# nekStab/neklab

Measured on AMD Instinct MI355X. Metric: linop matvecs/sec + Arnoldi iter time, E=10k N=7, 1/2/4/8 GPU, higher is better.
Workload: dtype f64

## Files before the change

neklab_amd/csrc/lns.hip:

```cpp
#include <cmath>
#include <functional>
#include <map>
#include <string>

#include "internal.h"

using namespace nlg;

namespace {

constexpr int NT = 256;
constexpr int NB = 512;

struct F3 {
    double *p[3];
};
struct CF3 {
    const double *p[3];
};
__device__ __forceinline__ int64_t lane_lo(int64_t ld) { return (int64_t)blockIdx.y * ld; }
__device__ __forceinline__ F3 lane_f3(F3 a, int64_t lo) {
#pragma unroll
    for (int c = 0; c < 3; ++c)
        if (a.p[c]) a.p[c] += lo;
// ... 1974 lines not shown
    hipStream_t st = m->ctx->stream;
    const int dim = m->dim, nl = L.nl;
    const int64_t ld = L.ld();
    const double dt = op->dt, b0 = op->adv_b0;
    double **unew = op->ubuf[2];
    NLG_LAUNCH(k_axpy1, lgrid(grid_for(m->lpn), nl), dim3(NT), 0, st, m->lpn, op->p, (const double *)op->pr_x, 1.0, ld);
    const bool fg = sem_opgradt_has_fg(m);
    NLG_TRY(sem_opgradt(m, op->pr_x, op->gp, fg, nullptr, nullptr, nl, ld, ld));
    NLG_TRY(sem_gs(m, op->gp, dim, nullptr, fg ? LAYOUT_FG : LAYOUT_NAT, nl, ld, 0));
    const bool fused = op->d_filt && op->filt_fused;
    if (!fused) {
        CF3 wt = {{m->d_mbinv[0], m->d_mbinv[1], m->d_mbinv[2]}};
        const bool wb = fg && op->maskb_v && m->d_maskb_fg && m->d_binv_fg;
        if (wb) wt.p[0] = m->d_binv_fg;
        if (fg)
            launch_nf(dim, k_axpy_w<1, true>, k_axpy_w<2, true>, k_axpy_w<3, true>, lgrid(grid_for(m->lvn), nl), st, m->lvn, f3(unew, dim), cf3(op->gp, dim),
                      wt, dt / b0, ld, (const int *)m->d_slot_fg, m->np1, wb ? (const unsigned char *)m->d_maskb_fg : (const unsigned char *)nullptr);
        else
            launch_nf(dim, k_axpy_w<1>, k_axpy_w<2>, k_axpy_w<3>, lgrid(grid_for(m->lvn), nl), st, m->lvn, f3(unew, dim), cf3(op->gp, dim), wt, dt / b0,
                      ld, (const int *)nullptr, 1, (const unsigned char *)nullptr);
    }
    if (op->d_filt) {
        double *fl[4] = {unew[0], unew[1], dim == 3 ? unew[2] : op->tbuf[0], op->tbuf[0]};
        const int nf = dim + (op->cfg.ifheat ? 1 : 0);
        if (fused)
            NLG_TRY(sem_filter(m, op->d_filt, fl, nf, nl, ld, op->gp, m->d_mbinv, dt / b0, fg ? (const int *)m->d_slot_fg : nullptr));
        else
            NLG_TRY(sem_filter(m, op->d_filt, fl, nf, nl, ld));
    }
    NLG_HIP(hipGetLastError());
    rotate3(op->ubuf);
    op->st_steps += nl;
    return 0;
}

int advance(const Lanes &L) {
    NLG_TRY(adv_a(L));
    NLG_TRY(helm_solve(L, L.op->adv_k, L.op->adv_h2));
    NLG_TRY(adv_b(L));
    NLG_TRY(pres_solve(L, L.op->dt / L.op->adv_b0));
    return adv_c(L);
}

int reset_state(nlg_linop *op, int nl) {
    nlg_mesh *m = op->mesh;
    NLG_TRY(slab_ensure(op, nl));
    lane_bind(op);
    const int64_t nlev = (int64_t)(6 * m->dim + (op->cfg.ifheat ? 6 : 0)) * m->lvs;
    for (int v = 0; v < nl; ++v) NLG_HIP(hipMemsetAsync(op->slab + (size_t)v * (size_t)op->slab_ld, 0, sizeof(double) * (size_t)nlev, m->ctx->stream));
    return 0;
}

int begin_run(nlg_linop *op, int nl) {
    NLG_TRY(reset_state(op, nl));
    op->istep = 0;
    op->nproj = 0;
    for (int v = 0; v < kMaxLanes; ++v) op->lane_viters[v] = op->lane_piters[v] = 0;
    op->orbit_end_valid = op->upo_fdot_valid = false;
    return 0;
}

int load_state(nlg_linop *op, int lane, const nlg_vec *v, int irst) {
    nlg_mesh *m = op->mesh;
    hipStream_t st = m->ctx->stream;
    for (int c = 0; c < m->dim; ++c)
        NLG_HIP(hipMemcpyAsync(at_lane(op, op->ubuf[0][c], lane), v->vel(c, irst), sizeof(double) * (size_t)m->lvn, hipMemcpyDeviceToDevice, st));
    NLG_HIP(hipMemcpyAsync(at_lane(op, op->p, lane), v->pr(irst), sizeof(double) * (size_t)m->lpn, hipMemcpyDeviceToDevice, st));
    if (op->cfg.ifheat)
        NLG_HIP(hipMemcpyAsync(at_lane(op, op->tbuf[0], lane), v->theta(0, irst), sizeof(double) * (size_t)m->lvn, hipMemcpyDeviceToDevice, st));
    return 0;
}

int store_state(nlg_linop *op, int lane, nlg_vec *v, int irst) {
    nlg_mesh *m = op->mesh;
    hipStream_t st = m->ctx->stream;
    for (int c = 0; c < m->dim; ++c)
        NLG_HIP(hipMemcpyAsync(v->vel(c, irst), at_lane(op, op->ubuf[0][c], lane), sizeof(double) * (size_t)m->lvn, hipMemcpyDeviceToDevice, st));
    NLG_HIP(hipMemcpyAsync(v->pr(irst), at_lane(op, op->p, lane), sizeof(double) * (size_t)m->lpn, hipMemcpyDeviceToDevice, st));
    if (op->cfg.ifheat)
        NLG_HIP(hipMemcpyAsync(v->theta(0, irst), at_lane(op, op->tbuf[0], lane), sizeof(double) * (size_t)m->lvn, hipMemcpyDeviceToDevice, st));
    return 0;
}

int state_minus_x0(nlg_linop *op, int lane, double c, nlg_vec *out) {
    nlg_mesh *m = op->mesh;
    const int dim = m->dim;
    DdtArgs A;
    memset(&A, 0, sizeof(A));
    for (int f = 0; f <= dim; ++f) {
        const bool pr = f == dim;
        A.out[f] = pr ? out->pr() : out->vel(f), A.n[f] = pr ? m->lpn : m->lvn;
        A.src[f][0] = at_lane(op, pr ? op->p : op->ubuf[0][f], lane), A.c[f][0] = c;
        A.src[f][1] = pr ? op->baseflow->pr() : op->baseflow->vel(f), A.c[f][1] = -c;
    }
    NLG_LAUNCH(k_bdf_ddt, dim3(grid_for(m->lvn), dim + 1), dim3(NT), 0, m->ctx->stream, A);
    NLG_HIP(hipGetLastError());
    return 0;
}

enum { FDOT_START = 0, FDOT_PRE, FDOT_END };
int capture_fdot(nlg_linop *op, int lane, int phase) {
    nlg_mesh *m = op->mesh;
    const int dim = m->dim;
    const double idt = 1.0 / op->dt;
    if (phase == FDOT_START) return state_minus_x0(op, lane, idt, op->upo_f0);
    nlg_vec *o = op->upo_fT;
    DdtArgs A;
    memset(&A, 0, sizeof(A));
    for (int c = 0; c < dim; ++c) A.out[c] = o->vel(c), A.n[c] = m->lvn;
    A.out[dim] = o->pr(), A.n[dim] = m->lpn;
    if (phase == FDOT_PRE) {
        const int k = std::min(op->nsteps, op->cfg.torder);
        for (int c = 0; c < dim; ++c)
            for (int j = 0; j < k; ++j) A.src[c][j] = at_lane(op, op->ubuf[j][c], lane), A.c[c][j] = -BDF_C[k][j] * idt;
    } else {
        const int k = std::min(op->nsteps, op->cfg.torder);
        A.acc = 1;
        for (int c = 0; c < dim; ++c) A.src[c][0] = at_lane(op, op->ubuf[0][c], lane), A.c[c][0] = BDF_B0[k] * idt;
        A.src[dim][0] = at_lane(op, op->pr_x, lane), A.c[dim][0] = idt;
        op->upo_fdot_valid = true;
    }
    NLG_LAUNCH(k_bdf_ddt, dim3(grid_for(m->lvn), dim + 1), dim3(NT), 0, m->ctx->stream, A);
    NLG_HIP(hipGetLastError());
    return 0;
}

template <typename Hook>
int run_steps(const Lanes &L, int fdot_lane, Hook after_step) {
    nlg_linop *op = L.op;
    for (int istep = 1; istep <= op->nsteps; ++istep) {
        if (fdot_lane >= 0 && istep == op->nsteps) NLG_TRY(capture_fdot(op, fdot_lane, FDOT_PRE));
        NLG_TRY(advance(L));
        if (fdot_lane >= 0 && istep == 1) NLG_TRY(capture_fdot(op, fdot_lane, FDOT_START));
        NLG_TRY(after_step(istep));
    }
    if (fdot_lane >= 0) NLG_TRY(capture_fdot(op, fdot_lane, FDOT_END));
    return 0;
}
int run_steps(const Lanes &L, int fdot_lane = -1) {
    return run_steps(L, fdot_lane, [](int) { return 0; });
}

int project_lines(nlg_linop *op, const ProjLines &P, int nf, F3 f, int s, unsigned mask) {
    nlg_mesh *m = op->mesh;
    hipStream_t st = m->ctx->stream;
    const int64_t nl = P.nlines, ld = op->slab_ld, tld = P.tld;
    const dim3 g((unsigned)((nl + NT / 64 - 1) / (NT / 64)), (unsigned)s);
    const int *off = P.off, *idx = P.idx, *gs = P.gslot;
    const double *cv = P.cv, *sv = P.sv, *iden = P.iden, *glob = P.glob;
    if (!gs) {
        launch_nf(nf, k_proj_alpha<1>, k_proj_alpha<2>, k_proj_alpha<3>, g, st, nl, off, idx, P.weight, cv, sv, tld, iden, f, ld, mask);
    } else {
        const int64_t cnt = P.nglob * s * 2 * nf;
        NLG_HIP(hipMemsetAsync(P.glob, 0, sizeof(double) * (size_t)cnt, st));
        if (nl > 0)
            launch_nf(nf, k_proj_sums<1>, k_proj_sums<2>, k_proj_sums<3>, g, st, nl, off, idx, gs, P.weight, cv, sv, tld,
                      CF3{{f.p[0], f.p[1], f.p[2]}}, ld, mask, P.glob);
        NLG_TRY(allreduce_sum(m->ctx, P.glob, (int)cnt));
        if (nl > 0) launch_nf(nf, k_proj_apply<1>, k_proj_apply<2>, k_proj_apply<3>, g, st, nl, off, idx, gs, cv, sv, tld, iden, glob, f, ld, mask);
    }
    NLG_HIP(hipGetLastError());
    return 0;
}

int project_alpha(nlg_linop *op, int s, int slot, unsigned mask) {
    if (op->proj_v.nlines == 0) return 0;
    NLG_TRY(project_lines(op, op->proj_v, op->mesh->dim, f3(op->ubuf[slot], op->mesh->dim), s, mask));
    const ProjLines &Pp = op->proj_p;
    if ((Pp.gslot || Pp.nlines > 0) && slot == 0) NLG_TRY(project_lines(op, Pp, 1, F3{{op->p, nullptr, nullptr}}, s, mask));
    return 0;
}

int do_matvec_block(nlg_linop *op, int s, const nlg_vec *const *vin, nlg_vec *const *vout, int adjoint) {
    NLG_CHECK(op && vin && vout, "exptA block matvec: NULL argument");
    NLG_CHECK(s >= 1 && s <= kMaxLanes, "exptA block matvec: %d vectors unsupported (1..%d)", s, kMaxLanes);
    NLG_CHECK(op->inited, "exptA block matvec: nlg_linop_init has not been called");
    NLG_NO_OTD(op, "exptA matvec");
    if (op->orbit) {
        NLG_CHECK(s <= kMaxLanes - 1, "exptA block matvec: orbit mode advances the base flow as one of the %d lanes, %d vectors unsupported (1..%d)",
                  kMaxLanes, s, kMaxLanes - 1);
        NLG_CHECK(!adjoint, "exptA rmatvec: orbit mode has no adjoint (the adjoint of a time-dependent linearisation needs U(T - t); nlg_linop_set_orbit)");
    }
    nlg_mesh *m = op->mesh;
    const int want_scal = op->cfg.ifheat ? 1 : 0;
    for (int v = 0; v < s; ++v) {
        NLG_CHECK(vin[v] && vout[v] && vin[v]->mesh == m && vout[v]->mesh == m, "exptA block matvec: vector %d NULL or on a different mesh", v);
        NLG_CHECK(vin[v]->nscal == want_scal && vout[v]->nscal == want_scal, "exptA block matvec: vector %d carries %d scalars, the operator %d", v,
                  vin[v]->nscal, want_scal);
        NLG_CHECK(op->cfg.no_history || (vin[v]->lorder >= op->cfg.torder && vout[v]->lorder >= op->cfg.torder), "exptA block matvec: vector lorder < time order");
        for (int u = 0; u < s; ++u) NLG_CHECK(vin[v] != vout[u], "exptA block matvec: an input vector is also an output vector");
        for (int u = 0; u < v; ++u) NLG_CHECK(vout[v] != vout[u], "exptA block matvec: the same output vector twice");
    }
    const int nrst = op->cfg.no_history ? 0 : op->cfg.torder - 1;
    const int nl = op->orbit ? s + 1 : s, lb = op->orbit ? s : -1;
    NLG_CHECK(op->proj_lanes == 0 || s <= op->proj_lanes, "exptA block matvec: %d vectors on an operator with %d wavenumber lanes (nlg_linop_set_projection_lanes)", s,
              op->proj_lanes);
    const unsigned all = (1u << s) - 1u;
    NLG_TRY(begin_run(op, nl));
    for (int v = 0; v < s; ++v) NLG_TRY(load_state(op, v, vin[v], 0));
    NLG_TRY(project_alpha(op, s, 0, all));
    if (lb >= 0) NLG_TRY(load_state(op, lb, op->baseflow, 0));
    Lanes L{op, nl, lb};
    L.adjoint = adjoint;
    NLG_TRY(run_steps(L, lb, [&](int istep) -> int {
        if (istep <= nrst) {
            unsigned replayed = 0;
            for (int v = 0; v < s; ++v)
                if (vin[v]->nrst > 0) {
                    NLG_TRY(load_state(op, v, vin[v], istep));
                    replayed |= 1u << v;
                }
            if (replayed) NLG_TRY(project_alpha(op, s, 0, replayed));
        }
        return 0;
    }));
    for (int slot = 0; slot < 3; ++slot) NLG_TRY(project_alpha(op, s, slot, all));
    for (int v = 0; v < s; ++v) {
        NLG_TRY(nlg_vec_zero(vout[v]));
        NLG_TRY(store_state(op, v, vout[v], 0));
    }
    if (lb >= 0) {
        NLG_TRY(nlg_vec_zero(op->orbit_end));
        NLG_TRY(store_state(op, lb, op->orbit_end, 0));
        op->orbit_end_valid = true;
    }
    for (int irst = 1; irst <= nrst; ++irst) {
        NLG_TRY(advance(L));
        for (int v = 0; v < s; ++v) {
            NLG_TRY(store_state(op, v, vout[v], irst));
            vout[v]->nrst = std::max(vout[v]->nrst, irst);
        }
    }
    op->st_matvecs += s;
    return 0;
}

int do_matvec(nlg_linop *op, const nlg_vec *vin, nlg_vec *vout, int adjoint) {
    NLG_CHECK(op && vin && vout, "exptA matvec: NULL argument");
    NLG_CHECK(op->inited, "exptA matvec: nlg_linop_init has not been called (reference: exptA%%init(), 1cyl.usr:20)");
    nlg_mesh *m = op->mesh;
    NLG_CHECK(vin->mesh == m && vout->mesh == m,
              "exptA matvec: vector on a different mesh (reference: type_error, exponential_propagator.f90:53-58)");
    NLG_CHECK(vin->nscal == (op->cfg.ifheat ? 1 : 0) && vout->nscal == vin->nscal,
              "exptA matvec: the vectors carry %d scalar(s), the operator expects %d (cfg.ifheat)", vin->nscal, op->cfg.ifheat ? 1 : 0);
    NLG_CHECK(op->cfg.no_history || (vin->lorder >= op->cfg.torder && vout->lorder >= op->cfg.torder),
              "exptA matvec: vector lorder %d < time order %d", vin->lorder, op->cfg.torder);
    NLG_CHECK(vin != vout, "exptA matvec: vec_in and vec_out must be distinct (intent(in) / intent(out))");
    return do_matvec_block(op, 1, &vin, &vout, adjoint);
}

int do_integrate_forced_block(nlg_linop *op, int s, const nlg_vec *const *ic, const nlg_vec *const *f_re, const nlg_vec *const *f_im, double omega,
                              int adjoint, nlg_vec *const *vout) {
    NLG_CHECK(op && f_re && vout, "integrate_forced: NULL argument");
    NLG_CHECK(s >= 1 && s <= kMaxLanes, "integrate_forced: %d forcings unsupported (1..%d)", s, kMaxLanes);
    NLG_CHECK(op->inited, "integrate_forced: nlg_linop_init has not been called");
    NLG_NO_OTD(op, "integrate_forced");
    NLG_CHECK(!op->orbit, "integrate_forced: not available in orbit mode (the forced response about a time-periodic base flow is not built; nlg_linop_set_orbit)");
    NLG_CHECK(op->proj_lanes == 0, "integrate_forced: not available on an operator with wavenumber lanes (a forced run does not project; nlg_linop_set_projection_lanes)");
    nlg_mesh *m = op->mesh;
    Lanes L{op, s};
    for (int v = 0; v < s; ++v) {
        NLG_CHECK(f_re[v] && vout[v], "integrate_forced: NULL argument (forcing or output of lane %d)", v);
        L.f_re[v] = f_re[v];
        L.f_im[v] = f_im ? f_im[v] : nullptr;
    }
    for (int v = 0; v < s; ++v) {
        const nlg_vec *icv = ic ? ic[v] : nullptr;
        NLG_CHECK(L.f_re[v]->mesh == m && vout[v]->mesh == m && (!icv || icv->mesh == m) && (!L.f_im[v] || L.f_im[v]->mesh == m),
                  "integrate_forced: vector on a different mesh");
        for (int u = 0; u < s; ++u)
            NLG_CHECK(vout[v] != L.f_re[u] && vout[v] != L.f_im[u] && !(ic && vout[v] == ic[u]), "integrate_forced: the output must be distinct from the inputs");
        for (int u = 0; u < v; ++u) NLG_CHECK(vout[v] != vout[u], "integrate_forced: the same output vector twice");
        NLG_CHECK(L.f_re[v]->nscal == 0 && vout[v]->nscal == 0, "integrate_forced: scalar (temperature) coupling is not built yet");
    }
    hipStream_t st = m->ctx->stream;
    NLG_TRY(begin_run(op, s));
    for (int v = 0; v < s; ++v) {
        NLG_HIP(hipMemsetAsync(at_lane(op, op->p, v), 0, sizeof(double) * (size_t)m->lps, st));
        if (ic && ic[v]) NLG_TRY(load_state(op, v, ic[v], 0));
    }
    L.adjoint = adjoint;
    L.omega = omega, L.sign = adjoint ? -1.0 : 1.0;
    NLG_TRY(run_steps(L));
    for (int v = 0; v < s; ++v) {
        NLG_TRY(nlg_vec_zero(vout[v]));
        NLG_TRY(store_state(op, v, vout[v], 0));
    }
    return 0;
}

int do_integrate_forced(nlg_linop *op, const nlg_vec *ic, const nlg_vec *f_re, const nlg_vec *f_im, double omega, int adjoint, nlg_vec *vout) {
    NLG_CHECK(op && f_re && vout, "integrate_forced: NULL argument");
    return do_integrate_forced_block(op, 1, &ic, &f_re, &f_im, omega, adjoint, &vout);
}

int do_nonlinear_map(nlg_linop *op, const nlg_vec *vin, nlg_vec *vout) {
    NLG_CHECK(op && vin && vout, "nonlinear_map: NULL argument");
    NLG_NO_OTD(op, "nonlinear_map");
    nlg_mesh *m = op->mesh;
    NLG_CHECK(vin->mesh == m && vout->mesh == m, "nonlinear_map: vector on a different mesh (reference: type_error, fixed_point.f90:31-36)");
    NLG_CHECK(vin->nscal == (op->cfg.ifheat ? 1 : 0) && vout->nscal == vin->nscal,
              "nonlinear_map: the vectors carry %d scalar(s), the operator expects %d (cfg.ifheat)", vin->nscal, op->cfg.ifheat ? 1 : 0);
    NLG_CHECK(vin != vout, "nonlinear_map: vec_in and vec_out must be distinct");
    NLG_CHECK(!op->orbit, "nonlinear_map: the operator is in orbit mode and holds X0 as its base flow (use a second operator, or nlg_linop_set_orbit(op, NULL, 0))");
    NLG_TRY(nlg_vec_copy(op->baseflow, vin));
// ... 787 lines not shown
```

neklab_amd/csrc/vec.hip:

```cpp
#include <algorithm>

#include "internal.h"

using namespace nlg;

namespace {

constexpr int NT = 256;

__device__ __forceinline__ double wave_sum(double v) {
#pragma unroll
    for (int o = 32; o > 0; o >>= 1) v += __shfl_down(v, o, 64);
    return v;
}

__device__ __forceinline__ double block_sum(double v, double *sm) {
    v = wave_sum(v);
    const int lane = threadIdx.x & 63, wid = threadIdx.x >> 6;
    __syncthreads();
    if (lane == 0) sm[wid] = v;
    __syncthreads();
    double r = 0.0;
    if (threadIdx.x == 0) {
        const int nw = (blockDim.x + 63) >> 6;
// ... 83 lines not shown
    const int64_t beg = blockIdx.x * per, end = (beg + per < n2) ? beg + per : n2;
    const int64_t off = (int64_t)c * lvs;
    double2 *w2 = reinterpret_cast<double2 *>(w + off);
    const double2 *v2 = reinterpret_cast<const double2 *>(v + off);
    const double2 *t2 = reinterpret_cast<const double2 *>(fT + off);
    const double2 *f2 = reinterpret_cast<const double2 *>(f0 + off);
    const double2 *m2 = reinterpret_cast<const double2 *>(bm1);
    double acc = 0.0;
    for (int64_t i = beg + threadIdx.x; i < end; i += NT) {
        const double2 vv = v2[i], tv = t2[i];
        double2 wv = w2[i];
        wv.x = __dadd_rn(__dadd_rn(wv.x, -vv.x), __dmul_rn(t, tv.x));
        wv.y = __dadd_rn(__dadd_rn(wv.y, -vv.y), __dmul_rn(t, tv.y));
        w2[i] = wv;
        if (ip) {
            const double2 fv = f2[i], mv = m2[i];
            acc += vv.x * fv.x * mv.x + vv.y * fv.y * mv.y;
        }
    }
    if (ip) {
        const double s = block_sum(acc, sm);
        if (threadIdx.x == 0) partial[c * nblk + blockIdx.x] = s;
    }
}

__global__ __launch_bounds__(NT) void k_reduce_rows(const double *partial, int nper, double *out, int accumulate,
                                                    double *out2) {
    __shared__ double sm[4];
    const double *p = partial + (int64_t)blockIdx.x * nper;
    double acc = 0.0;
    for (int i = threadIdx.x; i < nper; i += NT) acc += p[i];
    const double s = block_sum(acc, sm);
    if (threadIdx.x == 0) {
        out[blockIdx.x] = s;
        if (accumulate) out2[blockIdx.x] += s;
    }
}

template <int KB>
__global__ __launch_bounds__(NT) void k_block_dot(const double *V, int64_t vstride, int k, const double *w,
                                                  const double *bm1, int64_t lvs, int nblk, int nper,
                                                  double *partial) {
    __shared__ double sm[4 * KB];
    const int c = blockIdx.y;
    const int j0 = blockIdx.z * KB;
    const int kc = (k - j0 < KB) ? (k - j0) : KB;
    const int64_t n2 = lvs >> 1;
    const int64_t per = (n2 + nblk - 1) / nblk;
    const int64_t beg = blockIdx.x * per, end = (beg + per < n2) ? beg + per : n2;
    const double2 *w2 = reinterpret_cast<const double2 *>(w + c * lvs);
    const double2 *m2 = reinterpret_cast<const double2 *>(bm1);
    const double2 *v2[KB];
#pragma unroll
    for (int j = 0; j < KB; ++j) {
        const int jj = (j < kc) ? j : 0;
        v2[j] = reinterpret_cast<const double2 *>(V + (int64_t)(j0 + jj) * vstride + c * lvs);
    }
    double acc[KB];
#pragma unroll
    for (int j = 0; j < KB; ++j) acc[j] = 0.0;
    for (int64_t i = beg + threadIdx.x; i < end; i += NT) {
        const double2 wv = w2[i], mv = m2[i];
        const double x0 = wv.x * mv.x, x1 = wv.y * mv.y;
        double2 vv[KB];
#pragma unroll
        for (int j = 0; j < KB; ++j) vv[j] = v2[j][i];
#pragma unroll
        for (int j = 0; j < KB; ++j) acc[j] += vv[j].x * x0 + vv[j].y * x1;
    }
    const int lane = threadIdx.x & 63, wid = threadIdx.x >> 6;
#pragma unroll
    for (int j = 0; j < KB; ++j) {
        const double s = wave_sum(acc[j]);
        if (lane == 0) sm[wid * KB + j] = s;
    }
    __syncthreads();
    if (threadIdx.x < kc) {
        const int j = threadIdx.x;
        const double s = sm[j] + sm[KB + j] + sm[2 * KB + j] + sm[3 * KB + j];
        partial[(int64_t)(j0 + j) * nper + c * nblk + blockIdx.x] = s;
    }
}

template <int KMAX>
__global__ __launch_bounds__(NT) void k_block_axpy_dot(const double *__restrict__ V, int64_t vstride, int k,
                                                       const double *__restrict__ h, double *__restrict__ w,
                                                       const double *__restrict__ bm1, int64_t lvs, int64_t nv,
                                                       double *__restrict__ partial) {
    __shared__ double sh[KMAX];
    __shared__ double sm[4][KMAX];
    for (int j = threadIdx.x; j < KMAX; j += NT) sh[j] = j < k ? h[j] : 0.0;
    __syncthreads();
    double acc[KMAX];
#pragma unroll
    for (int j = 0; j < KMAX; ++j) acc[j] = 0.0;
    for (int64_t i = blockIdx.x * (int64_t)NT + threadIdx.x; i < nv; i += (int64_t)gridDim.x * NT) {
        double v[KMAX];
#pragma unroll
        for (int j = 0; j < KMAX; ++j) v[j] = j < k ? V[(int64_t)j * vstride + i] : 0.0;
        double s = 0.0;
#pragma unroll
        for (int j = 0; j < KMAX; ++j) s += sh[j] * v[j];
        const double wn = w[i] - s;
        w[i] = wn;
        const double x = wn * bm1[i % lvs];
#pragma unroll
        for (int j = 0; j < KMAX; ++j) acc[j] += v[j] * x;
    }
    const int lane = threadIdx.x & 63, wid = threadIdx.x >> 6;
#pragma unroll
    for (int j = 0; j < KMAX; ++j) {
        const double t = wave_sum(acc[j]);
        if (lane == 0) sm[wid][j] = t;
    }
    __syncthreads();
    if (threadIdx.x < k) {
        const int j = threadIdx.x;
        partial[(int64_t)j * gridDim.x + blockIdx.x] = (sm[0][j] + sm[1][j]) + (sm[2][j] + sm[3][j]);
    }
}

template <int KH>
__global__ __launch_bounds__(NT) void k_block_axpy_dot2(const double *__restrict__ V, int64_t vstride, int k,
                                                        const double *__restrict__ h, double *__restrict__ w,
                                                        const double *__restrict__ bm1, int64_t lvs, int64_t nv,
                                                        double *__restrict__ partial) {
    extern __shared__ double dyn2[];
    double *sh = dyn2;
    double *stash = dyn2 + 2 * KH;
    __shared__ double sm[4][2 * KH];
    for (int j = threadIdx.x; j < 2 * KH; j += NT) sh[j] = j < k ? h[j] : 0.0;
    __syncthreads();
    double acc0[KH], acc1[KH];
#pragma unroll
    for (int j = 0; j < KH; ++j) acc0[j] = 0.0, acc1[j] = 0.0;
    double *mine = stash + threadIdx.x;
    for (int64_t i = blockIdx.x * (int64_t)NT + threadIdx.x; i < nv; i += (int64_t)gridDim.x * NT) {
        double v[KH];
#pragma unroll
        for (int j = 0; j < KH; ++j) v[j] = KH + j < k ? V[(int64_t)(KH + j) * vstride + i] : 0.0;
        double s1 = 0.0;
#pragma unroll
        for (int j = 0; j < KH; ++j) {
            s1 += sh[KH + j] * v[j];
            mine[j * NT] = v[j];
        }
#pragma unroll
        for (int j = 0; j < KH; ++j) v[j] = V[(int64_t)j * vstride + i];
        double s0 = 0.0;
#pragma unroll
        for (int j = 0; j < KH; ++j) s0 += sh[j] * v[j];
        const double wn = w[i] - (s0 + s1);
        w[i] = wn;
        const double x = wn * bm1[i % lvs];
#pragma unroll
        for (int j = 0; j < KH; ++j) {
            acc0[j] += v[j] * x;
            acc1[j] += mine[j * NT] * x;
        }
    }
    const int lane = threadIdx.x & 63, wid = threadIdx.x >> 6;
#pragma unroll
    for (int j = 0; j < KH; ++j) {
        const double t0 = wave_sum(acc0[j]), t1 = wave_sum(acc1[j]);
        if (lane == 0) sm[wid][j] = t0, sm[wid][KH + j] = t1;
    }
    __syncthreads();
    if (threadIdx.x < k) {
        const int j = threadIdx.x;
        partial[(int64_t)j * gridDim.x + blockIdx.x] = (sm[0][j] + sm[1][j]) + (sm[2][j] + sm[3][j]);
    }
}

__global__ __launch_bounds__(NT) void k_block_axpy(const double *V, int64_t vstride, int k, const double *h, double *w,
                                                   int64_t n2, int nrst, int64_t blk2, int consistent, double sign,
                                                   const double *hh) {
    extern __shared__ double sh0[];
    double *sh1 = sh0 + k;
    for (int j = threadIdx.x; j < k; j += NT) {
        sh0[j] = h[j];
        sh1[j] = hh ? hh[j] : h[j];
    }
    __syncthreads();
    double2 *w2 = reinterpret_cast<double2 *>(w);
    for (int64_t i = blockIdx.x * (int64_t)NT + threadIdx.x; i < n2; i += (int64_t)gridDim.x * NT) {
        const double *sh = (hh && i >= blk2) ? sh1 : sh0;
        double s0 = 0.0, s1 = 0.0;
        const double2 *v = reinterpret_cast<const double2 *>(V) + i;
        const int64_t vs2 = vstride >> 1;
        int j = 0;
        for (; j + 8 <= k; j += 8) {
            double2 t[8];
#pragma unroll
            for (int u = 0; u < 8; ++u) t[u] = v[(int64_t)(j + u) * vs2];
#pragma unroll
            for (int u = 0; u < 8; ++u) {
                s0 += sh[j + u] * t[u].x;
                s1 += sh[j + u] * t[u].y;
            }
        }
        for (; j < k; ++j) {
            const double2 t = v[(int64_t)j * vs2];
            s0 += sh[j] * t.x;
            s1 += sh[j] * t.y;
        }
        double2 wv = w2[i];
        wv.x += sign * s0;
        wv.y += sign * s1;
        w2[i] = wv;
        for (int r = 1; r <= nrst; ++r) {
            double c0 = s0, c1 = s1;
            if (consistent) {
                c0 = c1 = 0.0;
                for (int jj = 0; jj < k; ++jj) {
                    const double2 t = v[(int64_t)jj * vs2 + r * blk2];
                    c0 += sh[jj] * t.x;
                    c1 += sh[jj] * t.y;
                }
            }
            double2 rv = w2[i + r * blk2];
            rv.x += sign * c0;
            rv.y += sign * c1;
            w2[i + r * blk2] = rv;
        }
    }
}

template <int KB, int S>
__global__ __launch_bounds__(NT) void k_block_dot_s(const double *V, int64_t vstride, int k, const double *W, int64_t wstride,
                                                    const double *bm1, int64_t lvs, int nblk, int nper, double *partial) {
    __shared__ double sm[4 * KB * S];
    const int c = blockIdx.y;
    const int j0 = blockIdx.z * KB;
    const int kc = (k - j0 < KB) ? (k - j0) : KB;
    const int64_t n2 = lvs >> 1;
    const int64_t per = (n2 + nblk - 1) / nblk;
    const int64_t beg = blockIdx.x * per, end = (beg + per < n2) ? beg + per : n2;
    const double2 *m2 = reinterpret_cast<const double2 *>(bm1);
    const double2 *v2[KB];
#pragma unroll
    for (int j = 0; j < KB; ++j) {
        const int jj = (j < kc) ? j : 0;
        v2[j] = reinterpret_cast<const double2 *>(V + (int64_t)(j0 + jj) * vstride + c * lvs);
    }
    double acc[KB][S];
#pragma unroll
    for (int j = 0; j < KB; ++j)
#pragma unroll
        for (int v = 0; v < S; ++v) acc[j][v] = 0.0;
    for (int64_t i = beg + threadIdx.x; i < end; i += NT) {
        const double2 mv = m2[i];
        double x0[S], x1[S];
#pragma unroll
        for (int v = 0; v < S; ++v) {
            const double2 wv = reinterpret_cast<const double2 *>(W + (int64_t)v * wstride + c * lvs)[i];
            x0[v] = wv.x * mv.x;
            x1[v] = wv.y * mv.y;
        }
        double2 vv[KB];
#pragma unroll
        for (int j = 0; j < KB; ++j) vv[j] = v2[j][i];
#pragma unroll
        for (int j = 0; j < KB; ++j)
#pragma unroll
            for (int v = 0; v < S; ++v) acc[j][v] += vv[j].x * x0[v] + vv[j].y * x1[v];
    }
    const int lane = threadIdx.x & 63, wid = threadIdx.x >> 6;
#pragma unroll
    for (int j = 0; j < KB; ++j)
#pragma unroll
        for (int v = 0; v < S; ++v) {
            const double t = wave_sum(acc[j][v]);
            if (lane == 0) sm[wid * KB * S + j * S + v] = t;
        }
    __syncthreads();
    if (threadIdx.x < kc * S) {
        const int q = threadIdx.x;
        const double t = (sm[q] + sm[KB * S + q]) + (sm[2 * KB * S + q] + sm[3 * KB * S + q]);
        partial[((int64_t)j0 * S + q) * nper + c * nblk + blockIdx.x] = t;
    }
}

template <int S>
__global__ __launch_bounds__(NT) void k_block_axpy_s(const double *V, int64_t vstride, int k, const double *h, const double *hh,
                                                     double *W, int64_t wstride, int64_t n2, int64_t blk2, double sign) {
    extern __shared__ double shs[];
    double *sh0 = shs, *sh1 = shs + (size_t)k * S;
    for (int j = threadIdx.x; j < k * S; j += NT) {
        sh0[j] = h[j];
        sh1[j] = hh ? hh[j] : h[j];
    }
    __syncthreads();
    const int64_t vs2 = vstride >> 1, ws2 = wstride >> 1;
    double2 *w2 = reinterpret_cast<double2 *>(W);
    for (int64_t i = blockIdx.x * (int64_t)NT + threadIdx.x; i < n2; i += (int64_t)gridDim.x * NT) {
        const double *sh = (hh && i >= blk2) ? sh1 : sh0;
        const double2 *v = reinterpret_cast<const double2 *>(V) + i;
        double s0[S], s1[S];
#pragma unroll
        for (int q = 0; q < S; ++q) s0[q] = s1[q] = 0.0;
        int j = 0;
        for (; j + 8 <= k; j += 8) {
            double2 t[8];
#pragma unroll
            for (int u = 0; u < 8; ++u) t[u] = v[(int64_t)(j + u) * vs2];
#pragma unroll
            for (int u = 0; u < 8; ++u)
// ... 557 lines not shown
    hipError_t e = hipMalloc(&b->d, bytes);
    if (e != hipSuccess) {
        delete b;
        set_error("nlg_basis_create: hipMalloc(%zu bytes) failed: %s", bytes, hipGetErrorString(e));
        return 1;
    }
    NLG_HIP(hipMemsetAsync(b->d, 0, bytes, mesh->ctx->stream));
    NLG_HIP(hipMalloc(&b->d_h, sizeof(double) * (size_t)(3 * nvec + 16)));
    NLG_HIP(hipMemsetAsync(b->d_h, 0, sizeof(double) * (size_t)(3 * nvec + 16), mesh->ctx->stream));
    NLG_TRY(reduce_ws_reserve(mesh->ctx, nvec + 8));
    b->views.resize(nvec);
    for (int i = 0; i < nvec; ++i) {
        nlg_vec *v = new nlg_vec();
        v->mesh = mesh;
        v->nscal = nscal;
        v->lorder = lorder;
        v->ncomp = ncomp;
        v->main_len = main_len;
        v->total_len = b->stride;
        v->d = b->d + (int64_t)i * b->stride;
        v->owns = false;
        b->views[i] = v;
    }
    *out = b;
    return 0;
}

int nlg_basis_destroy(nlg_basis *b) {
    if (!b) return 0;
    for (auto *v : b->views) delete v;
    if (b->d) hipFree(b->d);
    if (b->d_h) hipFree(b->d_h);
    if (b->d_hb) hipFree(b->d_hb);
    delete b;
    return 0;
}

int nlg_basis_vec(nlg_basis *b, int i, nlg_vec **out) {
    NLG_CHECK(b && out, "nlg_basis_vec: NULL argument");
    NLG_CHECK(i >= 0 && i < b->nvec, "nlg_basis_vec: index %d out of range [0,%d)", i, b->nvec);
    *out = b->views[i];
    return 0;
}

}

namespace nlg {

static int reduce_rows_all(nlg_ctx *ctx, int rows, int per, double *out, double *acc) {
    hipStream_t st = ctx->stream;
    if (ctx->distributed()) {
        NLG_LAUNCH(k_reduce_rows, dim3(rows), dim3(NT), 0, st, ctx->d_partial, per, out, 0, (double *)nullptr);
        NLG_TRY(allreduce_sum(ctx, out, rows));
        if (acc) NLG_LAUNCH(k_vadd, dim3((rows + 255) / 256), dim3(256), 0, st, acc, out, rows);
    } else {
        ++g_collectives;
        NLG_LAUNCH(k_reduce_rows, dim3(rows), dim3(NT), 0, st, ctx->d_partial, per, out, acc ? 1 : 0, acc);
    }
    return 0;
}

int basis_block_dot_dev(const nlg_basis *b, int k, const nlg_vec *w, double *d_out, double *d_acc) {
    nlg_ctx *ctx = b->mesh->ctx;
    const nlg_vec *v0 = b->views[0];
    constexpr int KB = 8;
    const int nblk = dot_nblk(v0);
    const int nper = nblk * v0->ncomp;
    NLG_TRY(reduce_ws_reserve(ctx, k));
    ProfScope ps(ctx, P_BLOCKDOT);
    NLG_LAUNCH(k_block_dot<KB>, dim3(nblk, v0->ncomp, (k + KB - 1) / KB), dim3(NT), 0, ctx->stream, b->d,
                       b->stride, k, w->d, b->mesh->d_bm1, b->mesh->lvs, nblk, nper, ctx->d_partial);
    NLG_TRY(reduce_rows_all(ctx, k, nper, d_out, d_acc));
    NLG_HIP(hipGetLastError());
    return 0;
}

int basis_block_axpy_dev(const nlg_basis *b, int k, const double *d_h, nlg_vec *w, double sign, const double *d_hh,
                         bool main_only) {
    nlg_ctx *ctx = b->mesh->ctx;
    const int64_t n2 = w->main_len / 2;
    ProfScope ps(ctx, P_BLOCKAXPY);
    if (g_axpby_consistent) {
        const int64_t n2all = main_only ? n2 : n2 * (1 + w->nrst);
        NLG_LAUNCH(k_block_axpy, dim3(grid_for(n2all)), dim3(NT), sizeof(double) * 2 * k, ctx->stream, b->d, b->stride,
                           k, d_h, w->d, n2all, 0, n2, 0, sign, d_hh);
    } else {
        NLG_LAUNCH(k_block_axpy, dim3(grid_for(n2)), dim3(NT), sizeof(double) * 2 * k, ctx->stream, b->d, b->stride, k,
                           d_h, w->d, n2, w->nrst, n2, 0, sign, (const double *)nullptr);
    }
    NLG_HIP(hipGetLastError());
    return 0;
}

int basis_cgs2_dev(nlg_basis *b, int k, nlg_vec *w) {
    nlg_ctx *ctx = b->mesh->ctx;
    double *h = b->d_h, *h2 = b->d_h + b->nvec + 8;
    if (k > 0) {
        NLG_TRY(basis_block_dot_dev(b, k, w, h, nullptr));
        if (g_axpby_consistent) {
            if (k >= 24) {
                const nlg_vec *v0 = b->views[0];
                const int kf = std::min(k, 128);
                const int k0 = k - kf;
                const int64_t nv = (int64_t)v0->ncomp * b->mesh->lvs;
                const int G = 256;
                NLG_TRY(reduce_ws_reserve(ctx, k));
                if (k0 > 0) NLG_TRY(basis_block_axpy_dev(b, k0, h, w, -1.0, nullptr, true));
                const double *Vf = b->d + (int64_t)k0 * b->stride;
                {
                    ProfScope ps(ctx, P_AXPYDOT);
                    if (kf > 64) {
                        constexpr size_t lds2 = sizeof(double) * (2 * 64 + 64 * NT);
                        static bool attr_set = false;
                        if (!attr_set) {
                            NLG_HIP(hipFuncSetAttribute(reinterpret_cast<const void *>(&k_block_axpy_dot2<64>), hipFuncAttributeMaxDynamicSharedMemorySize, (int)lds2));
                            attr_set = true;
                        }
                        NLG_LAUNCH(k_block_axpy_dot2<64>, dim3(G), dim3(NT), lds2, ctx->stream, Vf, b->stride, kf,
                                           (const double *)(h + k0), w->d, (const double *)b->mesh->d_bm1, b->mesh->lvs, nv, ctx->d_partial);
                    } else {
                        NLG_LAUNCH(k_block_axpy_dot<64>, dim3(G), dim3(NT), 0, ctx->stream, Vf, b->stride, kf,
                                           (const double *)(h + k0), w->d, (const double *)b->mesh->d_bm1, b->mesh->lvs, nv, ctx->d_partial);
                    }
                }
                {
                    ProfScope ps(ctx, P_BLOCKAXPY);
                    const int64_t np2 = (w->main_len - nv) / 2;
                    if (np2 > 0)
                        NLG_LAUNCH(k_block_axpy, dim3(grid_for(np2)), dim3(NT), sizeof(double) * 2 * kf, ctx->stream,
                                           Vf + nv, b->stride, kf, (const double *)(h + k0), w->d + nv, np2, 0, np2, 0, -1.0,
                                           (const double *)nullptr);
                }
                NLG_TRY(reduce_rows_all(ctx, kf, G, h2 + k0, h + k0));
                if (k0 > 0) NLG_TRY(basis_block_dot_dev(b, k0, w, h2, h));
            } else {
                NLG_TRY(basis_block_axpy_dev(b, k, h, w, -1.0, nullptr, true));
                NLG_TRY(basis_block_dot_dev(b, k, w, h2, h));
            }
            NLG_TRY(basis_block_axpy_dev(b, k, h2, w, -1.0, h, false));
        } else {
            NLG_TRY(basis_block_axpy_dev(b, k, h, w, -1.0));
            NLG_TRY(basis_block_dot_dev(b, k, w, h2, h));
            NLG_TRY(basis_block_axpy_dev(b, k, h2, w, -1.0));
        }
    }
    const int nblk = dot_nblk(w);
    NLG_LAUNCH(k_dot_partial, dim3(nblk, w->ncomp), dim3(NT), 0, ctx->stream, w->d, w->d, b->mesh->d_bm1,
                       b->mesh->lvs, nblk, ctx->d_partial);
    NLG_TRY(reduce_rows_all(ctx, 1, nblk * w->ncomp, h + k, nullptr));
    const int64_t n2 = w->main_len * (1 + w->nrst) / 2;
    NLG_LAUNCH(k_scal_dev, dim3(grid_for(n2)), dim3(NT), 0, ctx->stream, reinterpret_cast<double2 *>(w->d),
                       h + k, 0, n2);
    NLG_HIP(hipGetLastError());
    return 0;
}

int basis_cgs2_batch_dev(int s, nlg_basis *const *b, int k, nlg_vec *const *w) {
    nlg_basis *b0 = b[0];
    nlg_mesh *m = b0->mesh;
    nlg_ctx *ctx = m->ctx;
    hipStream_t st = ctx->stream;
    if (!b0->d_hb) NLG_HIP(hipMalloc(&b0->d_hb, sizeof(double) * ((size_t)2 * b0->nvec * 4 + 64)));
    double *H1 = b0->d_hb, *Q = H1 + (size_t)s * k, *H2 = b0->d_hb + (size_t)b0->nvec * 4 + 8;
    if (!g_axpby_consistent) {
        for (int l = 0; l < s; ++l) {
            NLG_TRY(basis_cgs2_dev(b[l], k, w[l]));
            if (k > 0) NLG_HIP(hipMemcpyAsync(H1 + (size_t)l * k, b[l]->d_h, sizeof(double) * k, hipMemcpyDeviceToDevice, st));
            NLG_HIP(hipMemcpyAsync(Q + l, b[l]->d_h + k, sizeof(double), hipMemcpyDeviceToDevice, st));
        }
        return 0;
    }
    LaneVW P;
    int nrst = 0;
    for (int l = 0; l < kMaxLanes; ++l) {
        const int u = l < s ? l : 0;
        P.V[l] = b[u]->d, P.w[l] = w[u]->d, P.nrst[l] = w[u]->nrst;
        nrst = std::max(nrst, w[u]->nrst);
    }
    const nlg_vec *v0 = b0->views[0];
    constexpr int KB = 8;
    const int nblk = dot_nblk(v0), nper = nblk * v0->ncomp;
    const int64_t n2 = v0->main_len / 2;
    NLG_TRY(reduce_ws_reserve(ctx, s * std::max(k, 1)));
    auto dot = [&](double *out, double *acc) -> int {
        ProfScope ps(ctx, P_BLOCKDOT);
        NLG_LAUNCH(k_lane_block_dot<KB>, dim3(nblk, v0->ncomp * s, (k + KB - 1) / KB), dim3(NT), 0, st, P, b0->stride, k, v0->ncomp,
                   (const double *)m->d_bm1, m->lvs, nblk, nper, ctx->d_partial);
        return reduce_rows_all(ctx, s * k, nper, out, acc);
    };
    auto axpy = [&](const double *h, const double *hh, bool main_only) -> int {
        ProfScope ps(ctx, P_BLOCKAXPY);
        const int64_t n2all = main_only ? n2 : n2 * (1 + nrst);
        NLG_LAUNCH(k_lane_block_axpy, dim3(grid_for(n2all), s), dim3(NT), sizeof(double) * 2 * k, st, P, b0->stride, k, h, hh, n2, (int)main_only, -1.0);
        return 0;
    };
    if (k > 0) {
        NLG_TRY(dot(H1, nullptr));
        NLG_TRY(axpy(H1, nullptr, true));
        NLG_TRY(dot(H2, H1));
        NLG_TRY(axpy(H2, H1, false));
    }
    NLG_LAUNCH(k_lane_dot_partial, dim3(nblk, v0->ncomp, s), dim3(NT), 0, st, P, (const double *)m->d_bm1, m->lvs, nblk, nper, ctx->d_partial);
    NLG_TRY(reduce_rows_all(ctx, s, nper, Q, nullptr));
    NLG_LAUNCH(k_lane_scal_dev, dim3(grid_for(n2 * (1 + nrst)), s), dim3(NT), 0, st, P, (const double *)Q, n2);
    NLG_HIP(hipGetLastError());
    return 0;
}

}

extern "C" {

int nlg_basis_cgs2_batch(int s, nlg_basis *const *b, int k, nlg_vec *const *w, double *h, int ldh, double *beta) {
    NLG_CHECK(b && w && h && beta, "nlg_basis_cgs2_batch: NULL argument");
    NLG_CHECK(s >= 1 && s <= kMaxLanes, "nlg_basis_cgs2_batch: %d lanes unsupported (1..%d)", s, kMaxLanes);
    for (int l = 0; l < s; ++l) NLG_CHECK(b[l] && w[l], "nlg_basis_cgs2_batch: NULL basis or vector in lane %d", l);
    NLG_CHECK(k >= 0 && k <= b[0]->nvec, "nlg_basis_cgs2_batch: k=%d out of range [0,%d]", k, b[0]->nvec);
// ... 217 lines not shown
```

Measured before the change: 24.34.

## Fuse CGS2 norm and scaling into block-axpy epilogues; trim output zeroing

Adds a dedicated four-sweep CGS2 path for k between 24 and 128. It computes the first projection with a dot-only variant of the axpy-dot kernel, then fuses the second axpy with the weighted norm reduction, and folds the normalization scaling into the axpy over the remaining (restart) region. This removes separate dot/scale passes over the vector. Separately, zeroing of output vectors before store_state now memsets only the regions not overwritten by the subsequent copies, rather than the whole vector. The risk is subtle reordering of reductions changing rounding, and more code paths to keep consistent.

```diff
diff --git a/neklab_amd/csrc/lns.hip b/neklab_amd/csrc/lns.hip
--- a/neklab_amd/csrc/lns.hip
+++ b/neklab_amd/csrc/lns.hip
@@ -2080,6 +2080,18 @@
     return 0;
 }
 
+int reset_for_store(nlg_linop *op, nlg_vec *v, int nrst) {
+    nlg_mesh *m = op->mesh;
+    hipStream_t st = m->ctx->stream;
+    v->nrst = 0;
+    const int64_t beg = (int64_t)(1 + nrst) * v->main_len;
+    if (beg < v->total_len) NLG_HIP(hipMemsetAsync(v->d + beg, 0, sizeof(double) * (size_t)(v->total_len - beg), st));
+    const int nstored = m->dim + (op->cfg.ifheat ? 1 : 0);
+    for (int r = 0; r <= nrst && nstored < v->ncomp; ++r)
+        NLG_HIP(hipMemsetAsync(v->d + r * v->main_len + (int64_t)nstored * m->lvs, 0, sizeof(double) * (size_t)((v->ncomp - nstored) * m->lvs), st));
+    return 0;
+}
+
 int state_minus_x0(nlg_linop *op, int lane, double c, nlg_vec *out) {
     nlg_mesh *m = op->mesh;
     const int dim = m->dim;
@@ -2214,11 +2226,11 @@
     }));
     for (int slot = 0; slot < 3; ++slot) NLG_TRY(project_alpha(op, s, slot, all));
     for (int v = 0; v < s; ++v) {
-        NLG_TRY(nlg_vec_zero(vout[v]));
+        NLG_TRY(reset_for_store(op, vout[v], nrst));
         NLG_TRY(store_state(op, v, vout[v], 0));
     }
     if (lb >= 0) {
-        NLG_TRY(nlg_vec_zero(op->orbit_end));
+        NLG_TRY(reset_for_store(op, op->orbit_end, 0));
         NLG_TRY(store_state(op, lb, op->orbit_end, 0));
         op->orbit_end_valid = true;
     }
diff --git a/neklab_amd/csrc/vec.hip b/neklab_amd/csrc/vec.hip
--- a/neklab_amd/csrc/vec.hip
+++ b/neklab_amd/csrc/vec.hip
@@ -189,15 +189,17 @@
     }
 }
 
-template <int KMAX>
+template <int KMAX, bool SUB = true>
 __global__ __launch_bounds__(NT) void k_block_axpy_dot(const double *__restrict__ V, int64_t vstride, int k,
                                                        const double *__restrict__ h, double *__restrict__ w,
                                                        const double *__restrict__ bm1, int64_t lvs, int64_t nv,
                                                        double *__restrict__ partial) {
-    __shared__ double sh[KMAX];
+    __shared__ double sh[SUB ? KMAX : 1];
     __shared__ double sm[4][KMAX];
-    for (int j = threadIdx.x; j < KMAX; j += NT) sh[j] = j < k ? h[j] : 0.0;
-    __syncthreads();
+    if constexpr (SUB) {
+        for (int j = threadIdx.x; j < KMAX; j += NT) sh[j] = j < k ? h[j] : 0.0;
+        __syncthreads();
+    }
     double acc[KMAX];
 #pragma unroll
     for (int j = 0; j < KMAX; ++j) acc[j] = 0.0;
@@ -205,11 +207,14 @@
         double v[KMAX];
 #pragma unroll
         for (int j = 0; j < KMAX; ++j) v[j] = j < k ? V[(int64_t)j * vstride + i] : 0.0;
-        double s = 0.0;
-#pragma unroll
-        for (int j = 0; j < KMAX; ++j) s += sh[j] * v[j];
-        const double wn = w[i] - s;
-        w[i] = wn;
+        double wn = w[i];
+        if constexpr (SUB) {
+            double s = 0.0;
+#pragma unroll
+            for (int j = 0; j < KMAX; ++j) s += sh[j] * v[j];
+            wn -= s;
+            w[i] = wn;
+        }
         const double x = wn * bm1[i % lvs];
 #pragma unroll
         for (int j = 0; j < KMAX; ++j) acc[j] += v[j] * x;
@@ -279,9 +284,12 @@
     }
 }
 
+enum { EPI_NONE = 0, EPI_NORM, EPI_SCALE };
+template <int EPI>
 __global__ __launch_bounds__(NT) void k_block_axpy(const double *V, int64_t vstride, int k, const double *h, double *w,
                                                    int64_t n2, int nrst, int64_t blk2, int consistent, double sign,
-                                                   const double *hh) {
+                                                   const double *hh, const double *bm1, int64_t lvs2, double *partial,
+                                                   const double *scl) {
     extern __shared__ double sh0[];
     double *sh1 = sh0 + k;
     for (int j = threadIdx.x; j < k; j += NT) {
@@ -290,6 +298,11 @@
     }
     __syncthreads();
     double2 *w2 = reinterpret_cast<double2 *>(w);
+    double a = 0.0, nrm = 0.0;
+    if constexpr (EPI == EPI_SCALE) {
+        const double sv = scl[0];
+        a = sv > 0.0 ? 1.0 / sqrt(sv) : 0.0;
+    }
     for (int64_t i = blockIdx.x * (int64_t)NT + threadIdx.x; i < n2; i += (int64_t)gridDim.x * NT) {
         const double *sh = (hh && i >= blk2) ? sh1 : sh0;
         double s0 = 0.0, s1 = 0.0;
@@ -314,7 +327,15 @@
         double2 wv = w2[i];
         wv.x += sign * s0;
         wv.y += sign * s1;
+        if constexpr (EPI == EPI_SCALE) {
+            wv.x = __dmul_rn(wv.x, a);
+            wv.y = __dmul_rn(wv.y, a);
+        }
         w2[i] = wv;
+        if constexpr (EPI == EPI_NORM) {
+            const double2 mv = reinterpret_cast<const double2 *>(bm1)[i % lvs2];
+            nrm += wv.x * wv.x * mv.x + wv.y * wv.y * mv.y;
+        }
         for (int r = 1; r <= nrst; ++r) {
             double c0 = s0, c1 = s1;
             if (consistent) {
@@ -330,6 +351,11 @@
             rv.y += sign * c1;
             w2[i + r * blk2] = rv;
         }
+    }
+    if constexpr (EPI == EPI_NORM) {
+        __shared__ double sm[4];
+        const double s = block_sum(nrm, sm);
+        if (threadIdx.x == 0) partial[blockIdx.x] = s;
     }
 }
 
@@ -1053,12 +1079,70 @@
     ProfScope ps(ctx, P_BLOCKAXPY);
     if (g_axpby_consistent) {
         const int64_t n2all = main_only ? n2 : n2 * (1 + w->nrst);
-        NLG_LAUNCH(k_block_axpy, dim3(grid_for(n2all)), dim3(NT), sizeof(double) * 2 * k, ctx->stream, b->d, b->stride,
-                           k, d_h, w->d, n2all, 0, n2, 0, sign, d_hh);
+        NLG_LAUNCH(k_block_axpy<EPI_NONE>, dim3(grid_for(n2all)), dim3(NT), sizeof(double) * 2 * k, ctx->stream, b->d, b->stride,
+                           k, d_h, w->d, n2all, 0, n2, 0, sign, d_hh, (const double *)nullptr, (int64_t)0, (double *)nullptr,
+                           (const double *)nullptr);
     } else {
-        NLG_LAUNCH(k_block_axpy, dim3(grid_for(n2)), dim3(NT), sizeof(double) * 2 * k, ctx->stream, b->d, b->stride, k,
-                           d_h, w->d, n2, w->nrst, n2, 0, sign, (const double *)nullptr);
-    }
+        NLG_LAUNCH(k_block_axpy<EPI_NONE>, dim3(grid_for(n2)), dim3(NT), sizeof(double) * 2 * k, ctx->stream, b->d, b->stride, k,
+                           d_h, w->d, n2, w->nrst, n2, 0, sign, (const double *)nullptr, (const double *)nullptr, (int64_t)0,
+                           (double *)nullptr, (const double *)nullptr);
+    }
+    NLG_HIP(hipGetLastError());
+    return 0;
+}
+
+static int axpy_dot_sweep(nlg_basis *b, const double *Vf, int kf, const double *hf, nlg_vec *w, int64_t nv, int G) {
+    nlg_ctx *ctx = b->mesh->ctx;
+    ProfScope ps(ctx, P_AXPYDOT);
+    if (kf > 64) {
+        constexpr size_t lds2 = sizeof(double) * (2 * 64 + 64 * NT);
+        static bool attr_set = false;
+        if (!attr_set) {
+            NLG_HIP(hipFuncSetAttribute(reinterpret_cast<const void *>(&k_block_axpy_dot2<64>), hipFuncAttributeMaxDynamicSharedMemorySize, (int)lds2));
+            attr_set = true;
+        }
+        NLG_LAUNCH(k_block_axpy_dot2<64>, dim3(G), dim3(NT), lds2, ctx->stream, Vf, b->stride, kf, hf, w->d,
+                   (const double *)b->mesh->d_bm1, b->mesh->lvs, nv, ctx->d_partial);
+    } else {
+        NLG_LAUNCH((k_block_axpy_dot<64, true>), dim3(G), dim3(NT), 0, ctx->stream, Vf, b->stride, kf, hf, w->d,
+                   (const double *)b->mesh->d_bm1, b->mesh->lvs, nv, ctx->d_partial);
+    }
+    return 0;
+}
+
+static int cgs2_four_sweeps(nlg_basis *b, int k, nlg_vec *w) {
+    nlg_ctx *ctx = b->mesh->ctx;
+    nlg_mesh *m = b->mesh;
+    double *h = b->d_h, *h2 = b->d_h + b->nvec + 8;
+    const int64_t nv = (int64_t)w->ncomp * m->lvs;
+    const int G = 256;
+    NLG_TRY(reduce_ws_reserve(ctx, k));
+    {
+        ProfScope ps(ctx, P_BLOCKDOT);
+        for (int j0 = 0; j0 < k; j0 += 64)
+            NLG_LAUNCH((k_block_axpy_dot<64, false>), dim3(G), dim3(NT), 0, ctx->stream, (const double *)(b->d + (int64_t)j0 * b->stride),
+                       b->stride, std::min(k - j0, 64), (const double *)nullptr, w->d, (const double *)m->d_bm1, m->lvs, nv,
+                       ctx->d_partial + (int64_t)j0 * G);
+        NLG_TRY(reduce_rows_all(ctx, k, G, h, nullptr));
+    }
+    NLG_TRY(axpy_dot_sweep(b, b->d, k, h, w, nv, G));
+    NLG_TRY(reduce_rows_all(ctx, k, G, h2, h));
+    const int64_t nv2 = nv / 2, nr2 = (w->main_len * (1 + w->nrst) - nv) / 2;
+    const int gn = grid_for(nv2);
+    {
+        ProfScope ps(ctx, P_BLOCKAXPY);
+        NLG_LAUNCH(k_block_axpy<EPI_NORM>, dim3(gn), dim3(NT), sizeof(double) * 2 * k, ctx->stream, b->d, b->stride, k, (const double *)h2,
+                   w->d, nv2, 0, nv2, 0, -1.0, (const double *)nullptr, (const double *)m->d_bm1, m->lvs / 2, ctx->d_partial,
+                   (const double *)nullptr);
+    }
+    NLG_TRY(reduce_rows_all(ctx, 1, gn, h + k, nullptr));
+    {
+        ProfScope ps(ctx, P_BLOCKAXPY);
+        NLG_LAUNCH(k_block_axpy<EPI_SCALE>, dim3(grid_for(nr2)), dim3(NT), sizeof(double) * 2 * k, ctx->stream, b->d + nv, b->stride, k,
+                   (const double *)h, w->d + nv, nr2, 0, nr2, 0, -1.0, (const double *)nullptr, (const double *)nullptr, (int64_t)0,
+                   (double *)nullptr, (const double *)(h + k));
+    }
+    NLG_LAUNCH(k_scal_dev, dim3(grid_for(nv2)), dim3(NT), 0, ctx->stream, reinterpret_cast<double2 *>(w->d), h + k, 0, nv2);
     NLG_HIP(hipGetLastError());
     return 0;
 }
@@ -1066,44 +1150,30 @@
 int basis_cgs2_dev(nlg_basis *b, int k, nlg_vec *w) {
     nlg_ctx *ctx = b->mesh->ctx;
     double *h = b->d_h, *h2 = b->d_h + b->nvec + 8;
+    if (g_axpby_consistent && k >= 24 && k <= 128) return cgs2_four_sweeps(b, k, w);
     if (k > 0) {
         NLG_TRY(basis_block_dot_dev(b, k, w, h, nullptr));
         if (g_axpby_consistent) {
-            if (k >= 24) {
+            if (k > 128) {
                 const nlg_vec *v0 = b->views[0];
-                const int kf = std::min(k, 128);
-                const int k0 = k - kf;
+                const int kf = 128, k0 = k - kf;
                 const int64_t nv = (int64_t)v0->ncomp * b->mesh->lvs;
                 const int G = 256;
                 NLG_TRY(reduce_ws_reserve(ctx, k));
-                if (k0 > 0) NLG_TRY(basis_block_axpy_dev(b, k0, h, w, -1.0, nullptr, true));
+                NLG_TRY(basis_block_axpy_dev(b, k0, h, w, -1.0, nullptr, true));
                 const double *Vf = b->d + (int64_t)k0 * b->stride;
-                {
-                    ProfScope ps(ctx, P_AXPYDOT);
-                    if (kf > 64) {
-                        constexpr size_t lds2 = sizeof(double) * (2 * 64 + 64 * NT);
-                        static bool attr_set = false;
-                        if (!attr_set) {
-                            NLG_HIP(hipFuncSetAttribute(reinterpret_cast<const void *>(&k_block_axpy_dot2<64>), hipFuncAttributeMaxDynamicSharedMemorySize, (int)lds2));
-                            attr_set = true;
-                        }
-                        NLG_LAUNCH(k_block_axpy_dot2<64>, dim3(G), dim3(NT), lds2, ctx->stream, Vf, b->stride, kf,
-                                           (const double *)(h + k0), w->d, (const double *)b->mesh->d_bm1, b->mesh->lvs, nv, ctx->d_partial);
-                    } else {
-                        NLG_LAUNCH(k_block_axpy_dot<64>, dim3(G), dim3(NT), 0, ctx->stream, Vf, b->stride, kf,
-                                           (const double *)(h + k0), w->d, (const double *)b->mesh->d_bm1, b->mesh->lvs, nv, ctx->d_partial);
-                    }
-                }
+                NLG_TRY(axpy_dot_sweep(b, Vf, kf, h + k0, w, nv, G));
                 {
                     ProfScope ps(ctx, P_BLOCKAXPY);
                     const int64_t np2 = (w->main_len - nv) / 2;
                     if (np2 > 0)
-                        NLG_LAUNCH(k_block_axpy, dim3(grid_for(np2)), dim3(NT), sizeof(double) * 2 * kf, ctx->stream,
-                                           Vf + nv, b->stride, kf, (const double *)(h + k0), w->d + nv, np2, 0, np2, 0, -1.0,
-                                           (const double *)nullptr);
+                        NLG_LAUNCH(k_block_axpy<EPI_NONE>, dim3(grid_for(np2)), dim3(NT), sizeof(double) * 2 * kf, ctx->stream,
+                                   Vf + nv, b->stride, kf, (const double *)(h + k0), w->d + nv, np2, 0, np2, 0, -1.0,
+                                   (const double *)nullptr, (const double *)nullptr, (int64_t)0, (double *)nullptr,
+                                   (const double *)nullptr);
                 }
                 NLG_TRY(reduce_rows_all(ctx, kf, G, h2 + k0, h + k0));
-                if (k0 > 0) NLG_TRY(basis_block_dot_dev(b, k0, w, h2, h));
+                NLG_TRY(basis_block_dot_dev(b, k0, w, h2, h));
             } else {
                 NLG_TRY(basis_block_axpy_dev(b, k, h, w, -1.0, nullptr, true));
                 NLG_TRY(basis_block_dot_dev(b, k, w, h2, h));
```

Measured after the change: 24.23. No clear change (-0.5%).
